# flatironinstitute/walnuts

Hardware: AMD Instinct MI355X
Metric: leapfrog grad-evals/sec (all chains) (higher is better)
Workload: dtype f64

## Files before the change

### include/walnuts_hip.h

```cpp
#ifndef WALNUTS_HIP_H
#define WALNUTS_HIP_H

#include <stdbool.h>
#include <stddef.h>
#include <stdint.h>

#ifdef __cplusplus
extern "C" {
#endif

#define WALNUTS_HIP_EXPORT __attribute__((visibility("default")))


typedef enum { generic = 0, config = 1, interrupt = 2 } WalnutpyErrorType;
typedef struct WalnutpyError WalnutpyError;
WALNUTS_HIP_EXPORT const char* walnutpie_get_error_message(const WalnutpyError* err);
WALNUTS_HIP_EXPORT WalnutpyErrorType walnutpie_get_error_type(const WalnutpyError* err);
WALNUTS_HIP_EXPORT void walnutpie_destroy_error(WalnutpyError* err);

typedef void (*PRINT_CALLBACK)(const char* msg, size_t len, bool bad);
typedef void (*STREAM_CALLBACK)(const char* data, size_t size);

typedef int (*WN_LOGP_CFUNC)(size_t size, const double* theta, double* grad, double* lp, void* data);
#define WN_REFERENCE_SAMPLING_PARAMS                                                                              \
// ... 266 lines not shown
WALNUTS_HIP_EXPORT int wn_engine_init_positions(wn_engine* e, uint64_t seed, uint32_t chain_offset, double scale,
                                                WalnutpyError** err);
WALNUTS_HIP_EXPORT int wn_engine_init_masses_from_grad(wn_engine* e, double smoothing, WalnutpyError** err);
WALNUTS_HIP_EXPORT int wn_engine_average_masses(wn_engine* e, WalnutpyError** err);
WALNUTS_HIP_EXPORT int wn_engine_get_masses(wn_engine* e, double* out , WalnutpyError** err);
WALNUTS_HIP_EXPORT int wn_engine_adapt_step(wn_engine* e, uint64_t seed, uint32_t chain_offset, WalnutpyError** err);
WALNUTS_HIP_EXPORT int wn_engine_adapt_step_with_normals(wn_engine* e, const double* normals, WalnutpyError** err);
WALNUTS_HIP_EXPORT int wn_engine_seed(wn_engine* e, uint64_t seed, uint32_t chain_offset, WalnutpyError** err);
WALNUTS_HIP_EXPORT int wn_engine_seed_reference_streams(wn_engine* e, uint64_t seed, WalnutpyError** err);
WALNUTS_HIP_EXPORT int wn_engine_set_variates(wn_engine* e, const double* normals, const double* uniforms,
                                              int u_per_chain, WalnutpyError** err);

WALNUTS_HIP_EXPORT int wn_engine_warmup_step(wn_engine* e, double* draws_dev, int64_t draws_stride,
                                             WalnutpyError** err);
WALNUTS_HIP_EXPORT int wn_engine_freeze(wn_engine* e, WalnutpyError** err);
WALNUTS_HIP_EXPORT int wn_engine_sample_step(wn_engine* e, double* draws_dev, int64_t draws_stride,
                                             WalnutpyError** err);
WALNUTS_HIP_EXPORT int wn_engine_warmup_steps(wn_engine* e, int transitions, double* draws_dev, int64_t draws_stride,
                                              int64_t draws_transition_stride, WalnutpyError** err);
WALNUTS_HIP_EXPORT int wn_engine_sample_steps(wn_engine* e, int transitions, double* draws_dev, int64_t draws_stride,
                                              int64_t draws_transition_stride, WalnutpyError** err);
WALNUTS_HIP_EXPORT int wn_engine_synchronize(wn_engine* e, WalnutpyError** err);
WALNUTS_HIP_EXPORT int wn_engine_check(wn_engine* e, WalnutpyError** err);

WALNUTS_HIP_EXPORT int wn_engine_get_positions(wn_engine* e, double* out , WalnutpyError** err);
WALNUTS_HIP_EXPORT int wn_engine_get_inv_mass(wn_engine* e, double* out , WalnutpyError** err);
WALNUTS_HIP_EXPORT int wn_engine_get_step_sizes(wn_engine* e, double* out , WalnutpyError** err);
WALNUTS_HIP_EXPORT int wn_engine_get_logp(wn_engine* e, double* out , WalnutpyError** err);
WALNUTS_HIP_EXPORT int wn_engine_get_min_micro(wn_engine* e, int32_t* out , WalnutpyError** err);
WALNUTS_HIP_EXPORT int wn_engine_get_depths(wn_engine* e, int32_t* out , WalnutpyError** err);
WALNUTS_HIP_EXPORT int wn_engine_get_grad_evals(wn_engine* e, int64_t* out , WalnutpyError** err);
WALNUTS_HIP_EXPORT int wn_engine_get_rng_draws(wn_engine* e, int32_t* out , WalnutpyError** err);
WALNUTS_HIP_EXPORT int wn_engine_get_failed_extensions(wn_engine* e, int32_t* out , WalnutpyError** err);
WALNUTS_HIP_EXPORT int wn_engine_get_adam(wn_engine* e, double* out , WalnutpyError** err);
WALNUTS_HIP_EXPORT int wn_engine_get_estimator(wn_engine* e, double* draw_mean, double* draw_ssd,
                                               double* score_mean, double* score_ssd, double* weights ,
                                               WalnutpyError** err);
WALNUTS_HIP_EXPORT int wn_engine_total_grad_evals(wn_engine* e, int64_t* out, WalnutpyError** err);

WALNUTS_HIP_EXPORT int wn_engine_rhat(wn_engine* e, double* rhat, WalnutpyError** err);
WALNUTS_HIP_EXPORT int wn_engine_lp_sums(wn_engine* e, double* out3, WalnutpyError** err);
WALNUTS_HIP_EXPORT int wn_engine_lp_sq_dev(wn_engine* e, double mean_of_means, double* out1, WalnutpyError** err);
WALNUTS_HIP_EXPORT int wn_engine_warmup_spread(wn_engine* e, double* max_rel_diff_step, double* max_rel_diff_mass,
                                               WalnutpyError** err);
WALNUTS_HIP_EXPORT int wn_engine_rhat_datasets(wn_engine* e, double* rhat , WalnutpyError** err);
WALNUTS_HIP_EXPORT int wn_engine_warmup_spread_datasets(wn_engine* e, double* max_rel_diff_step ,
                                                        double* max_rel_diff_mass , WalnutpyError** err);
WALNUTS_HIP_EXPORT int wn_engine_average_masses_datasets(wn_engine* e, WalnutpyError** err);
WALNUTS_HIP_EXPORT int wn_engine_warmup_sums(wn_engine* e, double* sum_log_step, double* colsum_log_mass ,
                                             WalnutpyError** err);
WALNUTS_HIP_EXPORT int wn_engine_warmup_max_rel(wn_engine* e, double sum_log_step,
                                                const double* colsum_log_mass , size_t total_chains,
                                                double* max_rel_diff_step, double* max_rel_diff_mass,
                                                WalnutpyError** err);

WALNUTS_HIP_EXPORT int wn_engine_lanes(const wn_engine* e);
WALNUTS_HIP_EXPORT int wn_engine_dim_padded(const wn_engine* e);
WALNUTS_HIP_EXPORT int wn_engine_is_streaming(const wn_engine* e);
WALNUTS_HIP_EXPORT int wn_engine_held_tiles(const wn_engine* e);
WALNUTS_HIP_EXPORT int wn_engine_workgroups(const wn_engine* e);
WALNUTS_HIP_EXPORT int wn_engine_chain_groups(const wn_engine* e);
WALNUTS_HIP_EXPORT int wn_engine_lds_vectors(const wn_engine* e);
WALNUTS_HIP_EXPORT int64_t wn_engine_iteration(const wn_engine* e);
WALNUTS_HIP_EXPORT void* wn_engine_stream(const wn_engine* e);
WALNUTS_HIP_EXPORT double* wn_engine_positions_device(const wn_engine* e);
WALNUTS_HIP_EXPORT int wn_engine_last_kernel_ms(wn_engine* e, float* ms, WalnutpyError** err);
// ... 60 lines not shown
```

### walnuts_amd/_ffi.py

```python
from __future__ import annotations

import ctypes as C
import os
import sys
from typing import Optional

_HERE = os.path.dirname(os.path.abspath(__file__))
DEFAULT_LIB = os.path.join(_HERE, "lib", "libwalnuts_hip.so")

_dp = C.POINTER(C.c_double)
_errpp = C.POINTER(C.c_void_p)
PRINT_CALLBACK = C.CFUNCTYPE(None, C.c_char_p, C.c_size_t, C.c_bool)


class WalnutsHipError(RuntimeError):
    pass


class Config(C.Structure):
    _fields_ = [
        ("max_trajectory_doublings", C.c_int32),
        ("max_step_halvings", C.c_int32),
        ("min_micro_steps", C.c_int32),
        ("device", C.c_int32),
# ... 114 lines not shown
    ("wn_engine_create_with_grouped_datasets", _i32,
     [C.POINTER(_vp), _i32, _i32, _dp, _dp, _dp, _i32p, _i32, _i64p, _i32, _sz, C.POINTER(Config), _errpp]),
    ("wn_engine_num_datasets", _i32, [_vp]),
    ("wn_engine_destroy", None, [_vp]),
    ("wn_engine_eval", _i32, [_vp, _dp, _dp, _dp, _errpp]),
    ("wn_engine_set_positions", _i32, [_vp, _dp, _errpp]),
    ("wn_engine_set_masses", _i32, [_vp, _dp, _errpp]),
    ("wn_engine_set_step_sizes", _i32, [_vp, _dp, _errpp]),
    ("wn_engine_init_positions", _i32, [_vp, _u64, _u32, _dbl, _errpp]),
    ("wn_engine_init_masses_from_grad", _i32, [_vp, _dbl, _errpp]),
    ("wn_engine_average_masses", _i32, [_vp, _errpp]),
    ("wn_engine_get_masses", _i32, [_vp, _dp, _errpp]),
    ("wn_engine_adapt_step", _i32, [_vp, _u64, _u32, _errpp]),
    ("wn_engine_adapt_step_with_normals", _i32, [_vp, _dp, _errpp]),
    ("wn_engine_seed", _i32, [_vp, _u64, _u32, _errpp]),
    ("wn_engine_seed_reference_streams", _i32, [_vp, _u64, _errpp]),
    ("wn_engine_set_variates", _i32, [_vp, _dp, _dp, _i32, _errpp]),
    ("wn_engine_warmup_step", _i32, [_vp, _vp, _i64, _errpp]),
    ("wn_engine_freeze", _i32, [_vp, _errpp]),
    ("wn_engine_sample_step", _i32, [_vp, _vp, _i64, _errpp]),
    ("wn_engine_warmup_steps", _i32, [_vp, _i32, _vp, _i64, _i64, _errpp]),
    ("wn_engine_sample_steps", _i32, [_vp, _i32, _vp, _i64, _i64, _errpp]),
    ("wn_engine_synchronize", _i32, [_vp, _errpp]),
    ("wn_engine_check", _i32, [_vp, _errpp]),
    ("wn_engine_get_positions", _i32, [_vp, _dp, _errpp]),
    ("wn_engine_get_inv_mass", _i32, [_vp, _dp, _errpp]),
    ("wn_engine_get_step_sizes", _i32, [_vp, _dp, _errpp]),
    ("wn_engine_get_logp", _i32, [_vp, _dp, _errpp]),
    ("wn_engine_get_min_micro", _i32, [_vp, _i32p, _errpp]),
    ("wn_engine_get_depths", _i32, [_vp, _i32p, _errpp]),
    ("wn_engine_get_grad_evals", _i32, [_vp, _i64p, _errpp]),
    ("wn_engine_get_rng_draws", _i32, [_vp, _i32p, _errpp]),
    ("wn_engine_get_failed_extensions", _i32, [_vp, _i32p, _errpp]),
    ("wn_engine_get_adam", _i32, [_vp, _dp, _errpp]),
    ("wn_engine_get_estimator", _i32, [_vp, _dp, _dp, _dp, _dp, _dp, _errpp]),
    ("wn_engine_total_grad_evals", _i32, [_vp, _i64p, _errpp]),
    ("wn_engine_rhat", _i32, [_vp, _dp, _errpp]),
    ("wn_engine_lp_sums", _i32, [_vp, _dp, _errpp]),
    ("wn_engine_lp_sq_dev", _i32, [_vp, _dbl, _dp, _errpp]),
    ("wn_engine_warmup_spread", _i32, [_vp, _dp, _dp, _errpp]),
    ("wn_engine_rhat_datasets", _i32, [_vp, _dp, _errpp]),
    ("wn_engine_warmup_spread_datasets", _i32, [_vp, _dp, _dp, _errpp]),
    ("wn_engine_average_masses_datasets", _i32, [_vp, _errpp]),
    ("wn_engine_warmup_sums", _i32, [_vp, _dp, _dp, _errpp]),
    ("wn_engine_warmup_max_rel", _i32, [_vp, _dbl, _dp, _sz, _dp, _dp, _errpp]),
    ("wn_engine_lanes", _i32, [_vp]),
    ("wn_engine_dim_padded", _i32, [_vp]),
    ("wn_engine_is_streaming", _i32, [_vp]),
    ("wn_engine_workgroups", _i32, [_vp]),
    ("wn_engine_chain_groups", _i32, [_vp]),
    ("wn_engine_held_tiles", _i32, [_vp]),
    ("wn_engine_lds_vectors", _i32, [_vp]),
    ("wn_engine_iteration", _i64, [_vp]),
    ("wn_engine_stream", _vp, [_vp]),
    ("wn_engine_positions_device", _vp, [_vp]),
    ("wn_engine_last_kernel_ms", _i32, [_vp, C.POINTER(C.c_float), _errpp]),
    ("wn_engine_timing_reset", _i32, [_vp, _errpp]),
    ("wn_engine_region_begin", _i32, [_vp, _errpp]),
    ("wn_engine_region_ms", _i32, [_vp, C.POINTER(C.c_float), C.POINTER(C.c_int), _errpp]),
    ("wn_engine_kernel_times", _i32, [_vp, C.POINTER(C.c_float), _i32, C.POINTER(C.c_int), _errpp]),
    ("wn_engine_set_stream", _i32, [_vp, _vp, _errpp]),
    ("wn_engine_wait_stream", _i32, [_vp, _vp, _errpp]),
    ("wn_engine_release_stream", _i32, [_vp, _vp, _errpp]),
    ("wn_engine_wait_event", _i32, [_vp, _vp, _errpp]),
    ("wn_lanes_for_dim", _i32, [_i32, _i32, _i32]),
    ("wn_lanes_for_model_dim", _i32, [_i32, _i32, _i32, _i32]),
# ... 59 lines not shown
```

### walnuts_amd/csrc/wn_engine.hip

```cpp
#include "wn_hip.h"

#include <algorithm>
#include <cmath>
#include <cstdlib>
#include <cstring>
#include <memory>
#include <random>
#include <sstream>
#include <stdexcept>
#include <string>
#include <utility>
#include <vector>

#include "../../include/walnuts_hip.h"
#include "wn_elementwise.h"
#include "wn_init.h"
#include "wn_launch.h"
#include "wn_monitor.h"
#include "wn_traj.h"

#include "wn_host.h"

struct ReferenceStreams {
  std::vector<std::mt19937_64> eng;
// ... 1139 lines not shown
  });
}
int wn_engine_get_logp(wn_engine* e, double* out, WalnutpyError** err) {
  return guarded(err, [&] {
    if (e == nullptr || out == nullptr) throw std::invalid_argument("null argument"); e->download(e->logp, out, e->C); });
}
int wn_engine_get_min_micro(wn_engine* e, int32_t* out, WalnutpyError** err) {
  return guarded(err, [&] {
    if (e == nullptr || out == nullptr) throw std::invalid_argument("null argument");
    if (e->frozen) {
      e->download(e->min_micro, out, e->C);
    } else {
      std::vector<double> mm(2 * e->C);
      e->download(e->mm_state, mm.data(), mm.size());
      for (size_t c = 0; c < e->C; ++c) {
        const long long est = std::llround(mm[2 * c] / mm[2 * c + 1] / e->cfg.max_macro_steps_target);
        out[c] = static_cast<int32_t>(std::max<long long>(est, e->cfg.min_micro_steps));
      }
    }
  });
}
int wn_engine_get_depths(wn_engine* e, int32_t* out, WalnutpyError** err) {
  return guarded(err, [&] {
    if (e == nullptr || out == nullptr) throw std::invalid_argument("null argument"); e->download(e->depth, out, e->C); });
}
int wn_engine_get_grad_evals(wn_engine* e, int64_t* out, WalnutpyError** err) {
  return guarded(err, [&] {
    if (e == nullptr || out == nullptr) throw std::invalid_argument("null argument"); e->download(e->grad_evals, out, e->C); });
}
int wn_engine_get_failed_extensions(wn_engine* e, int32_t* out, WalnutpyError** err) {
  return guarded(err, [&] {
    if (e == nullptr || out == nullptr) throw std::invalid_argument("null argument");
    e->download(e->failed_ext, out, e->C);
  });
}
int wn_engine_get_rng_draws(wn_engine* e, int32_t* out, WalnutpyError** err) {
  return guarded(err, [&] {
    if (e == nullptr || out == nullptr) throw std::invalid_argument("null argument"); e->download(e->rng_draws, out, e->C); });
}
int wn_engine_get_adam(wn_engine* e, double* out, WalnutpyError** err) {
  return guarded(err, [&] {
    if (e == nullptr || out == nullptr) throw std::invalid_argument("null argument"); e->download(e->adam, out, 6 * e->C); });
}
int wn_engine_get_estimator(wn_engine* e, double* dm, double* ds, double* sm, double* ss, double* w,
                            WalnutpyError** err) {
  return guarded(err, [&] {
    e->download_rows(e->draw_mean, dm);
    e->download_rows(e->draw_ssd, ds);
    e->download_rows(e->score_mean, sm);
    e->download_rows(e->score_ssd, ss);
    e->download(e->est_weight, w, 2 * e->C);
  });
}
int wn_engine_total_grad_evals(wn_engine* e, int64_t* out, WalnutpyError** err) {
  return guarded(err, [&] {
    e->use_device();
    HIP_OK(hipMemsetAsync(e->scratch64.p, 0, sizeof(unsigned long long), e->stream));
    hipLaunchKernelGGL(wn::sum_i64_kernel, dim3(std::min<size_t>(256, (e->C + 255) / 256)), dim3(256), 0, e->stream, e->grad_evals.p,
                       static_cast<int>(e->C), e->scratch64.p);
    HIP_OK(hipGetLastError());
    unsigned long long v = 0;
    HIP_OK(hipMemcpyAsync(&v, e->scratch64.p, sizeof(v), hipMemcpyDeviceToHost, e->stream));
    HIP_OK(hipStreamSynchronize(e->stream));
    *out = static_cast<int64_t>(v);
  });
}
// ... 286 lines not shown
```

### walnuts_amd/csrc/wn_traj.h

```cpp
#pragma once

#include "wn_hip.h"

#include <type_traits>

#include "wn_devmath.h"
#include "wn_models.h"
#include "wn_params.h"

namespace wn {

constexpr int kRedStride(int nw) { return 4 * nw; }
constexpr int kRedDoubles(int nw) { return 2 * kRedStride(nw); }
constexpr int kShiftDoubles(int nw) { return 2 * 2 * 8 * nw; }

struct LaneTables {
  double e2, rc, lc;
  __device__ __forceinline__ void load(int lane) {
    e2 = wnd::as_f64(wn_tab_exp2_bits[lane & 63]);
    rc = wnd::as_f64(wn_tab_rcp_bits[lane < 49 ? lane : 48]);
    lc = wnd::as_f64(wn_tab_logc_bits[lane < 49 ? lane : 48]);
  }
};
struct UniformTab {
// ... 467 lines not shown
          Q.est_weight[2 * chain] = discount * w_draw0 + 1;
          Q.est_weight[2 * chain + 1] = discount * w_score0 + 1;
        }
        if constexpr (Self::kParkScalars) {
          Q.mm_state[2 * chain] = fetch(k_s0) + static_cast<double>(1ll << depth);
          Q.mm_state[2 * chain + 1] = fetch(k_s1) + 1.0;
        } else {
          Q.mm_state[2 * chain] += static_cast<double>(1ll << depth);
          Q.mm_state[2 * chain + 1] += 1.0;
        }
#pragma unroll
        for (int i = 0; i < 6; ++i) Q.adam[6 * chain + i] = meta->adam[i];
      }
      if (!warm) {
        double* w = Q.lp_stats + 3ll * chain;
        double w0, w1, w2;
        if constexpr (Self::kParkScalars) {
          w0 = fetch(k_s0);
          w1 = fetch(k_s1);
          w2 = fetch(k_s2);
        } else {
          w0 = w[0];
          w1 = w[1];
          w2 = w[2];
        }
        const double n = w0 + 1;
        const double delta = lpsel - w1;
        const double mean = w1 + delta / n;
        w[0] = n;
        w[1] = mean;
        w[2] = w2 + delta * (lpsel - mean);
      }
      if (WN_UNLIKELY(Q.rng_mode == kRngBuffer && n_draw > Q.u_stride)) err |= static_cast<int>(kErrVariatesExhausted);
      Q.failed_ext[chain] = (err >> 8) & 1;
      err &= 0xff;
      if (WN_UNLIKELY(err != 0)) atomicOr(Q.error_flags, static_cast<uint32_t>(err));
      Q.logp_out[chain] = lpsel;
      Q.depth_out[chain] = err ? -1 : depth;
      if constexpr (Self::kParkScalars) {
        Q.grad_evals[chain] = static_cast<long long>(wnd::as_u64(fetch(k_ge))) + n_grad;
      } else {
        Q.grad_evals[chain] += n_grad;
      }
      Q.rng_draws[chain] = n_draw;
    }
  }

  __device__ __forceinline__ bool macro_step(bool fwd, double logp_start, double& logp_pos, double& logp_joint) {
    WN_PHASE(kPhRestart);
    self().macro_begin();
    double h = fwd ? step : -step;
    int n = min_micro;
    for (int halvings = 0; halvings < P.max_halvings; ++halvings, n *= 2, h *= 0.5) {
      if (halvings > 0) self().macro_retry();
      WN_PHASE(kPhLeapfrog);
      const double part = self().leapfrog(h, n);
      WN_PHASE(kPhEnergy);
      self().energy(part, logp_pos, logp_joint);
      if (halvings == 0) {
        if (P.warmup && wave == 0) adam_record(fabs(logp_start - logp_joint));
      }
      if (fabs(logp_start - logp_joint) <= max_error) {
        WN_PHASE(kPhReversible);
        const bool rev = self().reversible(h, n, logp_joint);
        if (rev) self().macro_commit();
        return rev;
      }
// ... 72 lines not shown
      if (fwd ? !hot_is_fw : !hot_is_bk) {
        if (dirty) flush_hot_end();
        const int* e = fwd ? a_fw : a_bk;
        self().get(e[0], kTh);
        self().get(e[1], kRh);
        self().get(e[2], kG);
        self().moving_end_replaced();
      }
      double h_cur = fwd ? a_lj_fw : a_lj_bk;

      const int nleaf = 1 << (depth - 1);
      int sp = 0;
      bool ok = true;
      int c_in_th = kHot, c_in_rh = kHot, c_sel = kHot;
      double c_w = 0.0, c_lpsel = 0.0;
      for (int i = 0; i < nleaf; ++i) {
        double leaf_lp, leaf_lj;
        {
          int far_th[3] = {-1, -1, -1}, far_rh[3] = {-1, -1, -1};
          int nfar = 0;
          if (i + 1 == nleaf) {
            far_th[0] = fwd ? a_bk[0] : a_fw[0];
            far_rh[0] = fwd ? a_bk[1] : a_fw[1];
            nfar = 1;
          }
          if ((i & 3) == 3) {
            stack_buffers(sp - 2, far_th[1], far_rh[1]);
            nfar = 2;
            if ((i & 7) == 7) {
              stack_buffers(sp - 3, far_th[2], far_rh[2]);
              nfar = 3;
            }
          }
          self().expect_far_ends(nfar, far_th, far_rh);
        }
        if (!macro_step(fwd, h_cur, leaf_lp, leaf_lj)) {
          ok = false;
          break;
        }
        if (P.warmup && wave == 0) adam_make_room();
        h_cur = leaf_lj;
        c_in_th = kHot;
        c_in_rh = kHot;
        c_sel = kHot;
        {
          double none = 0.0;
          c_w = leaf_weight(leaf_lj, sp, a_w, none);
        }
        c_lpsel = leaf_lp;
        for (int l = 0; (i >> l) & 1; ++l) {
          --sp;
          int s_in_th, s_in_rh, s_sel;
          double s_w, s_lpsel;
          stack_read(sp, s_in_th, s_in_rh, s_sel, s_w, s_lpsel);
          WN_PHASE(kPhUturn);
          if (uturn_against(s_in_th, s_in_rh, fwd)) {
            ok = false;
            break;
          }
          WN_PHASE(kPhCombine);
          const double total = uni(s_w + c_w);
          const bool update = uniform01() * total < c_w;
          const int n_sel = update ? c_sel : s_sel;
          const double n_lpsel = update ? c_lpsel : s_lpsel;
          release_unless(s_sel, s_in_th, s_in_rh, n_sel);
          release_unless(c_in_th, s_in_th, s_in_rh, n_sel);
          release_unless(c_in_rh, s_in_th, s_in_rh, n_sel);
// ... 96 lines not shown
__device__ __attribute__((noinline)) void momentum_normals_to_lds(WN_LDS double* slots, const WN_LDS double* tables,
                                                                  int tiles, int tid, uint64_t seed, uint32_t chain,
                                                                  uint32_t transition) {
  const LdsTables tab{tables};
#pragma unroll 2
  for (int k = 0; k < tiles; ++k) {
    double z0, z1;
    wnd::stream_normal_pair(seed, chain, transition, wnd::kStreamMomentum, static_cast<uint32_t>(k * L + tid), z0, z1, tab);
    v2f64 z;
    z[0] = z0;
    z[1] = z1;
    *reinterpret_cast<WN_LDS v2f64*>(slots + (k * L + tid) * 2) = z;
  }
}

template <class Model, int NW, bool FMA = false, int HOLD = 0>
struct TrajMem : TrajBase<TrajMem<Model, NW, FMA, HOLD>, Model, NW> {
  using Base = TrajBase<TrajMem<Model, NW, FMA, HOLD>, Model, NW>;
  using typename Base::Meta;
  using Base::P; using Base::arena; using Base::tid; using Base::chain; using Base::Dp; using Base::aux;
  using Base::n_grad; using Base::max_error; using Base::min_micro; using Base::w_draw0; using Base::w_score0;
  static constexpr int L = Base::L;
  static constexpr bool kHasStartState = true;
  static constexpr bool kZeroCopy = true;
  static constexpr bool kDeferObservation = false;
  static constexpr bool kParkScalars = false;
  using ST = StreamTraits<Model>;
  static constexpr bool kTwoPass = ST::kTwoPass;
  typename Model::Aux auxs[4];
  static constexpr bool kHold = HOLD > 0;
  static constexpr int kHeld = kHold ? 2 * HOLD : 1;
  double hth[kHeld], hrh[kHeld];
  bool held;
  static constexpr bool kTablesInLds = kHold;
  const WN_LDS double* tab_lds;
  WN_LDS double* edge_lds;
  WN_LDS double* edge_base;
  int edge_parity;
  double edge_vec;
  static constexpr int kEdgeDoubles = (HOLD > 0 ? HOLD : 1) * NW * 2;
  __device__ __forceinline__ void publish_edges() {
    if constexpr (kHold && ST::kHalo) {
      edge_parity ^= 1;
      edge_lds = edge_base + edge_parity * kEdgeDoubles;
#pragma unroll
      for (int k = 0; k < HOLD; ++k) {
        if (k < tiles) {
          if (this->lane == 0) edge_lds[(k * NW + this->wave) * 2] = hth[2 * k];
          if (this->lane == 63) edge_lds[(k * NW + this->wave) * 2 + 1] = hth[2 * k + 1];
        }
      }
      __syncthreads();
      static_assert(2 * (HOLD > 0 ? HOLD : 1) <= 64, "one lane per tile and side");
      const int l = this->lane, w = this->wave;
      const int k = l < HOLD ? l : l - HOLD;
      const bool left = l < HOLD, first = w == 0, last = w == NW - 1;
      int idx;
      bool have;
      if (left) {
        have = !first || k > 0;
        idx = !first ? (k * NW + w - 1) * 2 + 1 : ((k > 0 ? k - 1 : 0) * NW + NW - 1) * 2 + 1;
      } else {
        have = !last || k + 1 < tiles;
        idx = !last ? (k * NW + w + 1) * 2 : ((k + 1 < HOLD ? k + 1 : k) * NW) * 2;
      }
      have = have && l < 2 * HOLD && k < tiles;
// ... 26 lines not shown
      return GatherTab{this->tabs};
    }
  }

  double* cur[3];
  double* alt[3];
  double* work[3];
  double* tmp[3];
  int slot_buf[12];
  unsigned own;
  double* im_buf;
  const double* im;
  WN_LDS double* im_lds;
  static constexpr int kMaxPending = 3;
  const double* pend_th[kMaxPending];
  const double* pend_rh[kMaxPending];
  int pend_bth[kMaxPending], pend_brh[kMaxPending];
  double pend_hot[kMaxPending], pend_far[kMaxPending];
  int n_pend;
  int pend_mask;
  bool pend_valid;
  double ke_part;
  double ut_hot, ut_far;
  bool ut_valid;
  int tiles;

  __device__ __forceinline__ TrajMem(const Params& p, WN_LDS double* pool, WN_LDS Meta* m, WN_LDS double* r,
                                     WN_LDS double* bc, double* ar)
      : Base(p, pool, m, r, bc, ar) {
    im_buf = ar + static_cast<long long>(p.pool_total - p.pool_lds) * p.dim_padded;
    im = im_buf;
    own = 0u;
    held = false;
    ut_valid = false;
    ut_hot = ut_far = 0.0;
    im_lds = (p.im_in_lds & 1u) ? bc + 2 + kShiftDoubles(NW) : nullptr;
    tab_lds = nullptr;
    edge_lds = edge_base = nullptr;
    edge_parity = 0;
    edge_vec = 0.0;
    if constexpr (kTablesInLds) {
      WN_LDS double* tl = bc + 2 + kShiftDoubles(NW) + p.dim_padded;
      if (this->wave == 0) {
        LaneTables t;
        t.load(this->lane);
        tl[this->lane] = t.e2;
        tl[64 + this->lane] = t.rc;
        tl[128 + this->lane] = t.lc;
      }
      tab_lds = tl;
      edge_base = tl + kLdsTableDoubles;
      edge_lds = edge_base;
      __syncthreads();
    }
    n_pend = 0;
    pend_mask = 0;
    pend_valid = false;
    for (int r = 0; r < 12; ++r) slot_buf[r] = -1;
    for (int i = 0; i < 3; ++i) cur[i] = alt[i] = work[i] = tmp[i] = nullptr;
    ke_part = 0.0;
    tiles = p.dim_padded / (2 * L);
  }

  __device__ __forceinline__ static double mad(double a, double b, double c) {
    if constexpr (FMA) return __builtin_fma(a, b, c);
    return a * b + c;
  }
  struct TileCx {
    int base, D;
    __device__ __forceinline__ static double mad(double a, double b, double c) { return TrajMem::mad(a, b, c); }
    __device__ __forceinline__ int index(int j) const { return base + j; }
    __device__ __forceinline__ bool valid(int j) const { return base + j < D; }
    __device__ __forceinline__ int dim() const { return D; }
  };
  __device__ __forceinline__ int pair_offset(int k) const { return (k * L + tid) * 2; }
  __device__ __forceinline__ static v2f64 ld(const double* p) { return *reinterpret_cast<const v2f64*>(p); }
  __device__ __forceinline__ static void st(double* p, double a, double b) {
    v2f64 t;
    t[0] = a;
    t[1] = b;
    *reinterpret_cast<v2f64*>(p) = t;
  }
  __device__ __forceinline__ double* pool_ptr(int b) const { return arena + static_cast<long long>(b) * Dp; }
  __device__ __forceinline__ v2f64 mass_at(int o) const {
    if (im_lds != nullptr) return *reinterpret_cast<const WN_LDS v2f64*>(im_lds + o);
    return ld(im + o);
  }
  __device__ __forceinline__ void expect_far_ends(int n, const int* bth, const int* brh) {
    n_pend = 0;
    pend_mask = 0;
    pend_valid = false;
    if constexpr (!kTwoPass) {
      if (P.im_in_lds & 2u) n = 0;
#pragma unroll
      for (int k = 0; k < kMaxPending; ++k) {
        pend_bth[k] = -1;
        if (k < n && bth[k] >= 0) {
          pend_bth[k] = bth[k];
          pend_brh[k] = brh[k];
          pend_th[k] = pool_ptr(bth[k]);
          pend_rh[k] = pool_ptr(brh[k]);
          n_pend = k + 1;
          pend_mask |= 1 << k;
        }
      }
    }
  }
  __device__ __forceinline__ void copy(double* dst, const double* src) const {
    for (int k = 0; k < tiles; ++k) {
      const int o = pair_offset(k);
      const v2f64 t = ld(src + o);
      st(dst + o, t[0], t[1]);
    }
  }
  __device__ __forceinline__ double*& slot_ptr(int r) {
    return r < 3 ? cur[r] : r < 6 ? alt[r - 3] : r < 9 ? work[r - 6] : tmp[r - 9];
  }
  __device__ __forceinline__ void set_slot(int r, int b, bool owned) {
    slot_buf[r] = b;
    slot_ptr(r) = pool_ptr(b);
    own = owned ? (own | (1u << r)) : (own & ~(1u << r));
  }
  __device__ __forceinline__ void ensure_writable(int r0) {
#pragma unroll
    for (int r = r0; r < r0 + 3; ++r) {
      if (!((own >> r) & 1u)) set_slot(r, this->alloc(), true);
    }
  }
  static __device__ __forceinline__ int slot_of(Comp c) {
    return c == kTh ? 0 : c == kRh ? 1 : c == kG ? 2 : c == kTh0 ? 3 : 4;
  }
  __device__ __forceinline__ int put_new(Comp c) {
    const int r = slot_of(c);
    if ((own >> r) & 1u) {
      own &= ~(1u << r);
      return slot_buf[r];
    }
    const int b = this->alloc();
    if (c != kG) copy(pool_ptr(b), slot_ptr(r));
    return b;
  }
  __device__ __forceinline__ void get(int b, Comp c) {
    const int r = slot_of(c);
    if ((own >> r) & 1u) this->release(slot_buf[r]);
    set_slot(r, b, false);
    if (kHold && r < 2) held = false;
  }

  __device__ __forceinline__ void halo(const double* v, int o, const v2f64& t, double (&prev)[2], double (&next)[2]) const {
    prev[0] = prev[1] = next[0] = next[1] = 0.0;
    if constexpr (ST::kHalo) {
      prev[0] = o > 0 ? v[o - 1] : 0.0;
      prev[1] = t[0];
      next[0] = t[1];
      next[1] = o + 2 < Dp ? v[o + 2] : 0.0;
    }
  }
  __device__ __forceinline__ void load_mp(int o, double (&mp2)[2]) const {
    mp2[0] = mp2[1] = 1.0;
    if (Model::kUsesParams) {
      const v2f64 p0 = ld(P.model_params + o);
      mp2[0] = p0[0];
      mp2[1] = p0[1];
    }
  }
  __device__ __forceinline__ void finish_sums(double (&sums)[ST::kSums], typename Model::Aux& out) {
    if constexpr (ST::kHasSums) {
      double a = sums[0], b = ST::kSums > 1 ? sums[ST::kSums - 1] : 0.0;
      this->sum2(a, b);
      sums[0] = a;
      if (ST::kSums > 1) sums[ST::kSums - 1] = b;
      Model::stream_aux(sums, P.dim, this->uniform_tab(), out);
    }
  }
  __device__ __forceinline__ void aux_of(const double* theta, typename Model::Aux& out) {
    if constexpr (kTwoPass && ST::kHasSums) {
      double sums[ST::kSums];
      for (int i = 0; i < ST::kSums; ++i) sums[i] = 0.0;
      for (int k = 0; k < tiles; ++k) {
// ... 164 lines not shown
      ++n_grad;
    }
    ke_part = ke;
    if (!negate) {
      ut_valid = fuse;
      ut_hot = p_hot;
      ut_far = p_far;
      pend_valid = fuse;
    }
    return part;
  }
  __device__ __forceinline__ unsigned lane_bytes() const {
    return static_cast<unsigned>(this->wave * 64 + opaque_lane_id()) * 16u;
  }
  __device__ __forceinline__ static v2f64 ld_tile(const double* base, int k, unsigned lb) {
    return load_pair_at(opaque_scalar_pointer(base), lb + static_cast<unsigned>(k) * (L * 16u));
  }
  __device__ __forceinline__ static void st_tile(double* base, int k, unsigned lb, double x, double y) {
    v2f64 t;
    t[0] = x;
    t[1] = y;
    store_pair_at(opaque_scalar_pointer(base), lb + static_cast<unsigned>(k) * (L * 16u), t);
  }
  __device__ __forceinline__ v2f64 mass_tile(int k, unsigned lb) const {
    return *reinterpret_cast<const WN_LDS v2f64*>(reinterpret_cast<const WN_LDS char*>(im_lds) + k * (L * 16) + lb);
  }
  __device__ __forceinline__ void drop_held() {
    if constexpr (kHold) {
#pragma unroll
      for (int i = 0; i < kHeld; ++i) hth[i] = hrh[i] = 0.0;
      held = false;
    }
  }
  __device__ __forceinline__ void ensure_held() {
    if constexpr (kHold) {
      if (!held) {
        const unsigned lb = lane_bytes();
#pragma unroll
        for (int k = 0; k < HOLD; ++k) {
          if (k < tiles) {
            const v2f64 t0 = ld_tile(cur[0], k, lb), r0 = ld_tile(cur[1], k, lb);
            hth[2 * k] = t0[0];
            hth[2 * k + 1] = t0[1];
            hrh[2 * k] = r0[0];
            hrh[2 * k + 1] = r0[1];
          }
        }
        held = true;
      }
    }
  }
  struct TileLoads {
    v2f64 mp, av[kMaxPending], bv[kMaxPending];
  };
  template <int MASK>
  __device__ __forceinline__ void issue_tile(TileLoads& t, int k, unsigned lb) const {
    if (Model::kUsesParams) t.mp = ld_tile(P.model_params, k, lb);
#pragma unroll
    for (int q = 0; q < kMaxPending; ++q) {
      if ((MASK >> q) & 1) {
        t.av[q] = ld_tile(pend_th[q], k, lb);
        t.bv[q] = ld_tile(pend_rh[q], k, lb);
      }
    }
  }
  static constexpr int prefetch_tiles(int mask) {
    const int loads = (Model::kUsesParams ? 1 : 0) + 2 * ((mask & 1) + ((mask >> 1) & 1) + ((mask >> 2) & 1));
    if (loads == 0) return 1;
    const int sets = 16 / loads;
    return sets < 2 ? 1 : sets > 5 ? 4 : sets - 1;
  }
  template <int MASK, bool FUSE, bool STORE>
  __device__ __forceinline__ void held_step(double h, double& part, double& ke, double& p_hot, double& p_far) {
    const double half = 0.5 * h;
    const unsigned lb = lane_bytes();
    constexpr int PD = prefetch_tiles(MASK);
    TileLoads ring[PD + 1];
    v2f64 mass[2];
    part = 0.0;
    ke = 0.0;
    mass[0] = mass_tile(0, lb);
#pragma unroll
    for (int k = 0; k < PD; ++k) {
      if (k < tiles) issue_tile<MASK>(ring[k % (PD + 1)], k, lb);
    }
#pragma unroll
    for (int k = 0; k < HOLD; ++k) {
      if (k + PD < HOLD) {
        if (k + PD < tiles) issue_tile<MASK>(ring[(k + PD) % (PD + 1)], k + PD, lb);
      }
      if (k + 1 < HOLD) {
        if (k + 1 < tiles) mass[(k + 1) & 1] = mass_tile(k + 1, lb);
      }
      if (k < tiles) {
        const TileLoads& in = ring[k % (PD + 1)];
        const int o = pair_offset(k);
        const v2f64 m0 = mass[k & 1];
        const double t0[2] = {hth[2 * k], hth[2 * k + 1]}, r0[2] = {hrh[2 * k], hrh[2 * k + 1]};
        double th2[2] = {t0[0], t0[1]}, rh2[2] = {r0[0], r0[1]};
        double g2[2], mp2[2] = {1.0, 1.0};
        if (Model::kUsesParams) {
          mp2[0] = in.mp[0];
          mp2[1] = in.mp[1];
        }
        TileCx cx{o, P.dim};
        Model::grad(cx, th2, g2, mp2, aux);
#pragma unroll
        for (int j = 0; j < 2; ++j) rh2[j] = mad(half, g2[j], rh2[j]);
#pragma unroll
        for (int j = 0; j < 2; ++j) th2[j] = mad(h * m0[j], rh2[j], th2[j]);
        Model::eval(cx, th2, g2, mp2, aux, part);
#pragma unroll
        for (int j = 0; j < 2; ++j) rh2[j] = mad(half, g2[j], rh2[j]);
#pragma unroll
        for (int j = 0; j < 2; ++j) ke = mad(m0[j], rh2[j] * rh2[j], ke);
        if (FUSE) {
#pragma unroll
          for (int j = 0; j < 2; ++j) {
            const double sd = m0[j] * (th2[j] - t0[j]);
            p_hot = mad(rh2[j], sd, p_hot);
            p_far = mad(r0[j], sd, p_far);
          }
#pragma unroll
          for (int q = 0; q < kMaxPending; ++q) {
            if ((MASK >> q) & 1) {
#pragma unroll
              for (int j = 0; j < 2; ++j) {
                const double sd = m0[j] * (th2[j] - in.av[q][j]);
                pend_hot[q] = mad(rh2[j], sd, pend_hot[q]);
                pend_far[q] = mad(in.bv[q][j], sd, pend_far[q]);
              }
            }
          }
        }
        hth[2 * k] = th2[0];
        hth[2 * k + 1] = th2[1];
        hrh[2 * k] = rh2[0];
        hrh[2 * k + 1] = rh2[1];
      }
    }
    if (STORE) {
#pragma unroll
      for (int k = 0; k < HOLD; ++k) {
        if (k < tiles) {
          st_tile(alt[0], k, lb, hth[2 * k], hth[2 * k + 1]);
          st_tile(alt[1], k, lb, hrh[2 * k], hrh[2 * k + 1]);
        }
      }
    }
    ++n_grad;
  }
  __device__ __forceinline__ double leapfrog_two_pass_held(double h, int n) {
    const double half = 0.5 * h;
    const unsigned lb = lane_bytes();
    double part = 0.0, ke = 0.0;
    ensure_held();
    held = false;
    typename Model::Aux a_in = auxs[0], a_out = auxs[0];
    for (int s = 0; s < n; ++s) {
      double sums[ST::kSums];
#pragma unroll
      for (int i = 0; i < ST::kSums; ++i) sums[i] = 0.0;
      v2f64 mass[2];
      publish_edges();
      mass[0] = mass_tile(0, lb);
#pragma unroll
      for (int k = 0; k < HOLD; ++k) {
        if (k + 1 < HOLD) {
          if (k + 1 < tiles) mass[(k + 1) & 1] = mass_tile(k + 1, lb);
        }
        if (k < tiles) {
          const v2f64 m0 = mass[k & 1];
          double th2[2] = {hth[2 * k], hth[2 * k + 1]}, rh2[2] = {hrh[2 * k], hrh[2 * k + 1]};
          double g2[2], mp2[2] = {1.0, 1.0}, prev[2], next[2];
          halo_held(k, prev, next);
          if (Model::kUsesParams) {
            const v2f64 p0 = ld_tile(P.model_params, k, lb);
            mp2[0] = p0[0];
            mp2[1] = p0[1];
          }
// ... 35 lines not shown
          Model::stream_logp(cx, th2, prev, next, mp2, a_out, part);
#pragma unroll
          for (int j = 0; j < 2; ++j) rh2[j] = mad(half, g2[j], rh2[j]);
#pragma unroll
          for (int j = 0; j < 2; ++j) ke = mad(m0[j], rh2[j] * rh2[j], ke);
          hrh[2 * k] = rh2[0];
          hrh[2 * k + 1] = rh2[1];
        }
      }
      ++n_grad;
      a_in = a_out;
    }
#pragma unroll
    for (int k = 0; k < HOLD; ++k) {
      if (k < tiles) {
        st_tile(alt[0], k, lb, hth[2 * k], hth[2 * k + 1]);
        st_tile(alt[1], k, lb, hrh[2 * k], hrh[2 * k + 1]);
      }
    }
    auxs[1] = a_out;
    aux = a_out;
    ke_part = ke;
    ut_valid = false;
    return part;
  }
  __device__ __forceinline__ double leapfrog_held(double h, int n) {
    double part = 0.0, ke = 0.0, p_hot = 0.0, p_far = 0.0;
    const bool fuse = n == 1;
    const bool fwd = h > 0;
#pragma unroll
    for (int q = 0; q < kMaxPending; ++q) pend_hot[q] = pend_far[q] = 0.0;
    ensure_held();
    held = false;
    if (fuse) {
      switch (pend_mask) {
        case 0: held_step<0, true, true>(h, part, ke, p_hot, p_far); break;
        case 1: held_step<1, true, true>(h, part, ke, p_hot, p_far); break;
        case 2: held_step<2, true, true>(h, part, ke, p_hot, p_far); break;
        case 3: held_step<3, true, true>(h, part, ke, p_hot, p_far); break;
        case 4: held_step<4, true, true>(h, part, ke, p_hot, p_far); break;
        case 5: held_step<5, true, true>(h, part, ke, p_hot, p_far); break;
        case 6: held_step<6, true, true>(h, part, ke, p_hot, p_far); break;
        default: held_step<7, true, true>(h, part, ke, p_hot, p_far); break;
      }
    } else {
      for (int s = 1; s < n; ++s) held_step<0, false, false>(h, part, ke, p_hot, p_far);
      held_step<0, false, true>(h, part, ke, p_hot, p_far);
    }
    ke_part = ke;
    ut_valid = fuse;
    ut_hot = fwd ? p_hot : -p_hot;
    ut_far = fwd ? p_far : -p_far;
#pragma unroll
    for (int q = 0; q < kMaxPending; ++q) {
      pend_hot[q] = fwd ? pend_hot[q] : -pend_hot[q];
      pend_far[q] = fwd ? pend_far[q] : -pend_far[q];
    }
    pend_valid = fuse;
    return part;
  }
  __device__ __forceinline__ double leapfrog(double h, int n) {
    if constexpr (kTwoPass) {
      if constexpr (kHold) {
        ensure_writable(3);
        return leapfrog_two_pass_held(h, n);
      }
      return leapfrog_two_pass<0, 1>(false, h, n);
    } else {
      ensure_writable(3);
      if constexpr (kHold) return leapfrog_held(h, n);
      return leapfrog_sets(cur, alt, false, h, n);
    }
  }
  __device__ __forceinline__ void energy(double lp_partial, double& logp_pos, double& logp_joint) {
    double ke = ke_part;
    this->sum2(lp_partial, ke);
    logp_pos = uni(Model::finish(lp_partial, aux, P.dim));
    logp_joint = uni(logp_pos + (-0.5 * ke));
  }
  __device__ __forceinline__ void macro_begin() {}
  __device__ __forceinline__ void macro_retry() {}
  __device__ __forceinline__ void macro_commit() {
#pragma unroll
    for (int i = 0; i < 3; ++i) {
      double* t = cur[i];
      cur[i] = alt[i];
      alt[i] = t;
      const int b = slot_buf[i];
      slot_buf[i] = slot_buf[3 + i];
      slot_buf[3 + i] = b;
    }
    own = (own & ~0x3fu) | ((own & 0x7u) << 3) | ((own >> 3) & 0x7u);
    if constexpr (kHold) held = true;
    if constexpr (kTwoPass) {
      const typename Model::Aux t = auxs[0];
      auxs[0] = auxs[1];
      auxs[1] = t;
    }
  }
  __device__ __forceinline__ bool reversible(double h, int n, double logp_joint) {
    if (n == 1) return true;
    while (n >= 2 * min_micro) {
      n /= 2;
      h *= 2;
      double part;
      if constexpr (kTwoPass) {
        part = leapfrog_two_pass<1, 2>(true, h, n);
      } else {
        ensure_writable(6);
        part = leapfrog_sets(alt, work, true, h, n);
      }
      double lp, lj;
      energy(part, lp, lj);
      if (fabs(lj - logp_joint) <= max_error) return false;
    }
    return true;
  }

  __device__ __forceinline__ bool uturn_ptrs(const double* a, const double* b, bool fwd) {
    double p_hot = 0.0, p_far = 0.0;
    if constexpr (kHold) {
      ensure_held();
      const unsigned lb = lane_bytes();
      constexpr int PD = 4;
      v2f64 rm[PD + 1], ra[PD + 1], rb[PD + 1];
#pragma unroll
      for (int k = 0; k < PD; ++k) {
        if (k < tiles) {
          rm[k] = mass_tile(k, lb);
          ra[k] = ld_tile(a, k, lb);
          rb[k] = ld_tile(b, k, lb);
        }
      }
#pragma unroll
// ... 170 lines not shown
          halo_held(k, prev, next);
          if (Model::kUsesParams) {
            const v2f64 p0 = ld_tile(P.model_params, k, lb);
            mp2[0] = p0[0];
            mp2[1] = p0[1];
          }
          TileCx cx{pair_offset(k), P.dim};
          Model::stream_logp(cx, th2, prev, next, mp2, auxs[0], part);
        }
      }
    }
    WN_MARK(kPhEvaluated);
#pragma unroll
    for (int k = 0; k < HOLD; ++k) {
      if (k < tiles) {
        st_tile(cur[0], k, lb, hth[2 * k], hth[2 * k + 1]);
        st_tile(cur[1], k, lb, hrh[2 * k], hrh[2 * k + 1]);
      }
    }
    WN_MARK(kPhStored);
    held = true;
    ++n_grad;
    ke_part = ke;
    return part;
  }

  __device__ __forceinline__ double begin_transition(long long row, bool warm) {
    const wnd::SharedDivisor wd(w_draw0), ws(w_score0);
    im = warm ? im_buf : P.inv_mass + row;
    n_pend = 0;
    pend_mask = 0;
    pend_valid = false;
    drop_held();
    own = 0u;
    for (int r = 0; r < 12; ++r) slot_buf[r] = -1;
    ensure_writable(0);
    if constexpr (kHold) {
      if (im_lds != nullptr) return begin_transition_held(row, warm);
    }
    double part = 0.0, ke = 0.0;
    double sums[ST::kSums];
    for (int i = 0; i < ST::kSums; ++i) sums[i] = 0.0;
    for (int k = 0; k < tiles; ++k) {
      const int o = pair_offset(k);
      const v2f64 t0 = ld(P.theta + row + o);
      double th2[2] = {t0[0], t0[1]}, g2[2], mp2[2] = {1.0, 1.0}, m2[2], ch2[2], z2[2];
      if (Model::kUsesParams) {
        const v2f64 p0 = ld(P.model_params + o);
        mp2[0] = p0[0];
        mp2[1] = p0[1];
      }
      if (warm) {
        const v2f64 ds = ld(P.est_draw_ssd + row + o), ss = ld(P.est_score_ssd + row + o);
#pragma unroll
        for (int j = 0; j < 2; ++j) {
          m2[j] = __builtin_sqrt((ds[j] / wd) / (ss[j] / ws));
          ch2[j] = __builtin_sqrt(1.0 / m2[j]);
        }
        if (im_lds == nullptr) st(im_buf + o, m2[0], m2[1]);
      } else {
        const v2f64 m0 = ld(P.inv_mass + row + o), c0 = ld(P.chol_mass + row + o);
        m2[0] = m0[0]; m2[1] = m0[1];
        ch2[0] = c0[0]; ch2[1] = c0[1];
      }
      if (im_lds != nullptr) {
        v2f64 mm;
// ... 217 lines not shown
```

### walnuts_amd/engine.py

```python
from __future__ import annotations

import ctypes as C
from typing import Optional

import numpy as np

from . import _ffi

MODEL_STD_NORMAL, MODEL_DIAG_NORMAL, MODEL_FUNNEL, MODEL_RW1 = 0, 1, 2, 3
MODEL_LINEAR_REGRESSION, MODEL_LOGISTIC_REGRESSION = 4, 5
MODEL_HIER_LINEAR_REGRESSION, MODEL_HIER_LOGISTIC_REGRESSION = 15, 16
MODEL_HIER_LINEAR_REGRESSION_CENTERED, MODEL_HIER_LOGISTIC_REGRESSION_CENTERED = 17, 18
MODEL_POISSON_REGRESSION, MODEL_NEG_BINOMIAL_REGRESSION, MODEL_LINEAR_REGRESSION_SIGMA = 24, 25, 26
MODEL_HIER_POISSON_REGRESSION, MODEL_HIER_POISSON_REGRESSION_CENTERED = 27, 28
_dp = _ffi._dp


def default_config(lib_path: Optional[str] = None, **overrides) -> _ffi.Config:
    cfg = _ffi.Config()
    _ffi.load_library(lib_path).wn_default_config(C.byref(cfg))
    for k, v in overrides.items():
        if not hasattr(cfg, k):
            raise AttributeError(k)
        setattr(cfg, k, v)
# ... 218 lines not shown
        self._call(fn, out.ctypes.data_as(ptr))
        return out

    def positions(self):
        return self._get(self.lib.wn_engine_get_positions, (self.C, self.D))

    def masses(self):
        return self._get(self.lib.wn_engine_get_masses, (self.C, self.D))

    def inv_mass(self):
        return self._get(self.lib.wn_engine_get_inv_mass, (self.C, self.D))

    def step_sizes(self):
        return self._get(self.lib.wn_engine_get_step_sizes, (self.C,))

    def logp(self):
        return self._get(self.lib.wn_engine_get_logp, (self.C,))

    def adam(self):
        return self._get(self.lib.wn_engine_get_adam, (self.C, 6))

    def min_micro(self):
        return self._get(self.lib.wn_engine_get_min_micro, (self.C,), np.int32, _ffi._i32p)

    def depths(self):
        return self._get(self.lib.wn_engine_get_depths, (self.C,), np.int32, _ffi._i32p)

    def grad_evals(self):
        return self._get(self.lib.wn_engine_get_grad_evals, (self.C,), np.int64, _ffi._i64p)

    def failed_extensions(self):
        return self._get(self.lib.wn_engine_get_failed_extensions, (self.C,), np.int32, _ffi._i32p)

    def rng_draws(self):
        return self._get(self.lib.wn_engine_get_rng_draws, (self.C,), np.int32, _ffi._i32p)

    def estimator(self):
        dm, ds, sm, ss = (np.empty((self.C, self.D)) for _ in range(4))
        w = np.empty((self.C, 2))
        self._call(self.lib.wn_engine_get_estimator, *(x.ctypes.data_as(_dp) for x in (dm, ds, sm, ss, w)))
        return dict(draw_mean=dm, draw_ssd=ds, score_mean=sm, score_ssd=ss, weights=w)

    def total_grad_evals(self) -> int:
        v = C.c_int64()
        self._call(self.lib.wn_engine_total_grad_evals, C.byref(v))
        return v.value

    def last_kernel_ms(self) -> float:
        v = C.c_float()
        self._call(self.lib.wn_engine_last_kernel_ms, C.byref(v))
        return v.value

    def rhat(self) -> float:
        v = C.c_double()
        self._call(self.lib.wn_engine_rhat, C.cast(C.byref(v), _dp))
        return v.value

    def lp_sums(self):
        out = np.zeros(3)
        self._call(self.lib.wn_engine_lp_sums, out.ctypes.data_as(_dp))
        return out

    def lp_sq_dev(self, mean_of_means: float) -> float:
        v = C.c_double()
        self._call(self.lib.wn_engine_lp_sq_dev, mean_of_means, C.cast(C.byref(v), _dp))
        return v.value
# ... 98 lines not shown
```

Measured before the change: 1.029 billion.

## Defer storing held leaf state on odd leaves and replay when needed

```diff
diff --git a/include/walnuts_hip.h b/include/walnuts_hip.h
--- a/include/walnuts_hip.h
+++ b/include/walnuts_hip.h
@@ -322,6 +322,7 @@
 WALNUTS_HIP_EXPORT int wn_engine_get_grad_evals(wn_engine* e, int64_t* out , WalnutpyError** err);
 WALNUTS_HIP_EXPORT int wn_engine_get_rng_draws(wn_engine* e, int32_t* out , WalnutpyError** err);
 WALNUTS_HIP_EXPORT int wn_engine_get_failed_extensions(wn_engine* e, int32_t* out , WalnutpyError** err);
+WALNUTS_HIP_EXPORT int wn_engine_get_held_replays(wn_engine* e, int32_t* out , WalnutpyError** err);
 WALNUTS_HIP_EXPORT int wn_engine_get_adam(wn_engine* e, double* out , WalnutpyError** err);
 WALNUTS_HIP_EXPORT int wn_engine_get_estimator(wn_engine* e, double* draw_mean, double* draw_ssd,
                                                double* score_mean, double* score_ssd, double* weights ,
diff --git a/walnuts_amd/_ffi.py b/walnuts_amd/_ffi.py
--- a/walnuts_amd/_ffi.py
+++ b/walnuts_amd/_ffi.py
@@ -170,6 +170,7 @@
     ("wn_engine_get_grad_evals", _i32, [_vp, _i64p, _errpp]),
     ("wn_engine_get_rng_draws", _i32, [_vp, _i32p, _errpp]),
     ("wn_engine_get_failed_extensions", _i32, [_vp, _i32p, _errpp]),
+    ("wn_engine_get_held_replays", _i32, [_vp, _i32p, _errpp]),
     ("wn_engine_get_adam", _i32, [_vp, _dp, _errpp]),
     ("wn_engine_get_estimator", _i32, [_vp, _dp, _dp, _dp, _dp, _dp, _errpp]),
     ("wn_engine_total_grad_evals", _i32, [_vp, _i64p, _errpp]),
diff --git a/walnuts_amd/csrc/wn_engine.hip b/walnuts_amd/csrc/wn_engine.hip
--- a/walnuts_amd/csrc/wn_engine.hip
+++ b/walnuts_amd/csrc/wn_engine.hip
@@ -1195,6 +1195,14 @@
   return guarded(err, [&] {
     if (e == nullptr || out == nullptr) throw std::invalid_argument("null argument");
     e->download(e->failed_ext, out, e->C);
+    for (size_t c = 0; c < e->C; ++c) out[c] &= 1;
+  });
+}
+int wn_engine_get_held_replays(wn_engine* e, int32_t* out, WalnutpyError** err) {
+  return guarded(err, [&] {
+    if (e == nullptr || out == nullptr) throw std::invalid_argument("null argument");
+    e->download(e->failed_ext, out, e->C);
+    for (size_t c = 0; c < e->C; ++c) out[c] >>= 1;
   });
 }
 int wn_engine_get_rng_draws(wn_engine* e, int32_t* out, WalnutpyError** err) {
diff --git a/walnuts_amd/csrc/wn_traj.h b/walnuts_amd/csrc/wn_traj.h
--- a/walnuts_amd/csrc/wn_traj.h
+++ b/walnuts_amd/csrc/wn_traj.h
@@ -523,7 +523,9 @@
         w[2] = w2 + delta * (lpsel - mean);
       }
       if (WN_UNLIKELY(Q.rng_mode == kRngBuffer && n_draw > Q.u_stride)) err |= static_cast<int>(kErrVariatesExhausted);
-      Q.failed_ext[chain] = (err >> 8) & 1;
+      int note = (err >> 8) & 1;
+      if constexpr (Self::kZeroCopy) note |= self().replays() << 1;
+      Q.failed_ext[chain] = note;
       err &= 0xff;
       if (WN_UNLIKELY(err != 0)) atomicOr(Q.error_flags, static_cast<uint32_t>(err));
       Q.logp_out[chain] = lpsel;
@@ -662,7 +664,7 @@
               nfar = 3;
             }
           }
-          self().expect_far_ends(nfar, far_th, far_rh);
+          self().expect_far_ends(nfar, far_th, far_rh, (i & 1) != 0);
         }
         if (!macro_step(fwd, h_cur, leaf_lp, leaf_lj)) {
           ok = false;
@@ -825,6 +827,14 @@
   static constexpr int kHeld = kHold ? 2 * HOLD : 1;
   double hth[kHeld], hrh[kHeld];
   bool held;
+  static constexpr bool kDefer = kHold && !ST::kTwoPass;
+  unsigned cur_mem;
+  bool defer_leaf;
+  bool cand_stored;
+  double last_h, rp_h;
+  int last_n, rp_n;
+  int n_replay;
+  __device__ __forceinline__ int replays() const { return kDefer ? n_replay : 0; }
   static constexpr bool kTablesInLds = kHold;
   const WN_LDS double* tab_lds;
   WN_LDS double* edge_lds;
@@ -917,6 +927,12 @@
     im = im_buf;
     own = 0u;
     held = false;
+    cur_mem = 3u;
+    defer_leaf = false;
+    cand_stored = true;
+    last_h = rp_h = 0.0;
+    last_n = rp_n = 0;
+    n_replay = 0;
     ut_valid = false;
     ut_hot = ut_far = 0.0;
     im_lds = (p.im_in_lds & 1u) ? bc + 2 + kShiftDoubles(NW) : nullptr;
@@ -971,7 +987,8 @@
     if (im_lds != nullptr) return *reinterpret_cast<const WN_LDS v2f64*>(im_lds + o);
     return ld(im + o);
   }
-  __device__ __forceinline__ void expect_far_ends(int n, const int* bth, const int* brh) {
+  __device__ __forceinline__ void expect_far_ends(int n, const int* bth, const int* brh, bool odd_leaf) {
+    defer_leaf = odd_leaf;
     n_pend = 0;
     pend_mask = 0;
     pend_valid = false;
@@ -1017,6 +1034,9 @@
   }
   __device__ __forceinline__ int put_new(Comp c) {
     const int r = slot_of(c);
+    if constexpr (kDefer) {
+      if (r < 2 && !((cur_mem >> r) & 1u)) store_held(r == 0, r == 1);
+    }
     if ((own >> r) & 1u) {
       own &= ~(1u << r);
       return slot_buf[r];
@@ -1029,7 +1049,10 @@
     const int r = slot_of(c);
     if ((own >> r) & 1u) this->release(slot_buf[r]);
     set_slot(r, b, false);
-    if (kHold && r < 2) held = false;
+    if (kHold && r < 2) {
+      held = false;
+      cur_mem |= 1u << r;
+    }
   }
 
   __device__ __forceinline__ void halo(const double* v, int o, const v2f64& t, double (&prev)[2], double (&next)[2]) const {
@@ -1260,9 +1283,71 @@
       held = false;
     }
   }
+  __device__ __forceinline__ void store_held(bool th, bool rh) {
+    if constexpr (kHold) {
+      const unsigned lb = lane_bytes();
+      if (th) {
+#pragma unroll
+        for (int k = 0; k < HOLD; ++k) {
+          if (k < tiles) st_tile(cur[0], k, lb, hth[2 * k], hth[2 * k + 1]);
+        }
+        cur_mem |= 1u;
+      }
+      if (rh) {
+#pragma unroll
+        for (int k = 0; k < HOLD; ++k) {
+          if (k < tiles) st_tile(cur[1], k, lb, hrh[2 * k], hrh[2 * k + 1]);
+        }
+        cur_mem |= 2u;
+      }
+    }
+  }
+  __device__ __forceinline__ void store_candidate() {
+    if constexpr (kHold) {
+      const unsigned lb = lane_bytes();
+#pragma unroll
+      for (int k = 0; k < HOLD; ++k) {
+        if (k < tiles) {
+          st_tile(alt[0], k, lb, hth[2 * k], hth[2 * k + 1]);
+          st_tile(alt[1], k, lb, hrh[2 * k], hrh[2 * k + 1]);
+        }
+      }
+      cand_stored = true;
+    }
+  }
+  __device__ __forceinline__ void replay_unstored_leaf() {
+    if constexpr (kDefer) {
+      const unsigned lb = lane_bytes();
+#pragma unroll
+      for (int k = 0; k < HOLD; ++k) {
+        if (k < tiles) {
+          const v2f64 t0 = ld_tile(work[0], k, lb), r0 = ld_tile(work[1], k, lb);
+          hth[2 * k] = t0[0];
+          hth[2 * k + 1] = t0[1];
+          hrh[2 * k] = r0[0];
+          hrh[2 * k + 1] = r0[1];
+        }
+      }
+      const typename Model::Aux kept = aux;
+      const long long counted = n_grad;
+      double part, ke, p_hot = 0.0, p_far = 0.0;
+      for (int s = 0; s < rp_n; ++s) held_step<0, false>(rp_h, part, ke, p_hot, p_far);
+      n_grad = counted;
+      aux = kept;
+      store_held(!(cur_mem & 1u), !(cur_mem & 2u));
+      ++n_replay;
+    }
+  }
   __device__ __forceinline__ void ensure_held() {
     if constexpr (kHold) {
       if (!held) {
+        if constexpr (kDefer) {
+          if (WN_UNLIKELY(cur_mem != 3u)) {
+            replay_unstored_leaf();
+            held = true;
+            return;
+          }
+        }
         const unsigned lb = lane_bytes();
 #pragma unroll
         for (int k = 0; k < HOLD; ++k) {
@@ -1298,7 +1383,7 @@
     const int sets = 16 / loads;
     return sets < 2 ? 1 : sets > 5 ? 4 : sets - 1;
   }
-  template <int MASK, bool FUSE, bool STORE>
+  template <int MASK, bool FUSE>
   __device__ __forceinline__ void held_step(double h, double& part, double& ke, double& p_hot, double& p_far) {
     const double half = 0.5 * h;
     const unsigned lb = lane_bytes();
@@ -1365,15 +1450,6 @@
         hth[2 * k + 1] = th2[1];
         hrh[2 * k] = rh2[0];
         hrh[2 * k + 1] = rh2[1];
-      }
-    }
-    if (STORE) {
-#pragma unroll
-      for (int k = 0; k < HOLD; ++k) {
-        if (k < tiles) {
-          st_tile(alt[0], k, lb, hth[2 * k], hth[2 * k + 1]);
-          st_tile(alt[1], k, lb, hrh[2 * k], hrh[2 * k + 1]);
-        }
       }
     }
     ++n_grad;
@@ -1475,21 +1551,24 @@
     for (int q = 0; q < kMaxPending; ++q) pend_hot[q] = pend_far[q] = 0.0;
     ensure_held();
     held = false;
+    last_h = h;
+    last_n = n;
+    cand_stored = false;
     if (fuse) {
       switch (pend_mask) {
-        case 0: held_step<0, true, true>(h, part, ke, p_hot, p_far); break;
-        case 1: held_step<1, true, true>(h, part, ke, p_hot, p_far); break;
-        case 2: held_step<2, true, true>(h, part, ke, p_hot, p_far); break;
-        case 3: held_step<3, true, true>(h, part, ke, p_hot, p_far); break;
-        case 4: held_step<4, true, true>(h, part, ke, p_hot, p_far); break;
-        case 5: held_step<5, true, true>(h, part, ke, p_hot, p_far); break;
-        case 6: held_step<6, true, true>(h, part, ke, p_hot, p_far); break;
-        default: held_step<7, true, true>(h, part, ke, p_hot, p_far); break;
+        case 0: held_step<0, true>(h, part, ke, p_hot, p_far); break;
+        case 1: held_step<1, true>(h, part, ke, p_hot, p_far); break;
+        case 2: held_step<2, true>(h, part, ke, p_hot, p_far); break;
+        case 3: held_step<3, true>(h, part, ke, p_hot, p_far); break;
+        case 4: held_step<4, true>(h, part, ke, p_hot, p_far); break;
+        case 5: held_step<5, true>(h, part, ke, p_hot, p_far); break;
+        case 6: held_step<6, true>(h, part, ke, p_hot, p_far); break;
+        default: held_step<7, true>(h, part, ke, p_hot, p_far); break;
       }
     } else {
-      for (int s = 1; s < n; ++s) held_step<0, false, false>(h, part, ke, p_hot, p_far);
-      held_step<0, false, true>(h, part, ke, p_hot, p_far);
-    }
+      for (int s = 0; s < n; ++s) held_step<0, false>(h, part, ke, p_hot, p_far);
+    }
+    if (!(kDefer && defer_leaf && cur_mem == 3u)) store_candidate();
     ke_part = ke;
     ut_valid = fuse;
     ut_hot = fwd ? p_hot : -p_hot;
@@ -1510,6 +1589,9 @@
       }
       return leapfrog_two_pass<0, 1>(false, h, n);
     } else {
+      if constexpr (kDefer) {
+        if (cur_mem != 3u && held) swap_sets<1, 2>();
+      }
       ensure_writable(3);
       if constexpr (kHold) return leapfrog_held(h, n);
       return leapfrog_sets(cur, alt, false, h, n);
@@ -1535,6 +1617,11 @@
     }
     own = (own & ~0x3fu) | ((own & 0x7u) << 3) | ((own >> 3) & 0x7u);
     if constexpr (kHold) held = true;
+    if constexpr (kDefer) {
+      cur_mem = cand_stored ? 3u : 0u;
+      rp_h = last_h;
+      rp_n = last_n;
+    }
     if constexpr (kTwoPass) {
       const typename Model::Aux t = auxs[0];
       auxs[0] = auxs[1];
@@ -1543,6 +1630,9 @@
   }
   __device__ __forceinline__ bool reversible(double h, int n, double logp_joint) {
     if (n == 1) return true;
+    if constexpr (kDefer) {
+      if (n >= 2 * min_micro && !cand_stored) store_candidate();
+    }
     while (n >= 2 * min_micro) {
       n /= 2;
       h *= 2;
@@ -1779,6 +1869,10 @@
     pend_mask = 0;
     pend_valid = false;
     drop_held();
+    cur_mem = 3u;
+    defer_leaf = false;
+    cand_stored = true;
+    n_replay = 0;
     own = 0u;
     for (int r = 0; r < 12; ++r) slot_buf[r] = -1;
     ensure_writable(0);
diff --git a/walnuts_amd/engine.py b/walnuts_amd/engine.py
--- a/walnuts_amd/engine.py
+++ b/walnuts_amd/engine.py
@@ -274,6 +274,9 @@
     def failed_extensions(self):
         return self._get(self.lib.wn_engine_get_failed_extensions, (self.C,), np.int32, _ffi._i32p)
 
+    def held_replays(self):
+        return self._get(self.lib.wn_engine_get_held_replays, (self.C,), np.int32, _ffi._i32p)
+
     def rng_draws(self):
         return self._get(self.lib.wn_engine_get_rng_draws, (self.C,), np.int32, _ffi._i32p)
 
```

After: 1.031 billion (median of 6 runs). Within noise of the previous version (+0.2%).
